# stephaneguindon/phyml

Measured on AMD Instinct MI355X. Metric: M partial-lk site-updates/sec on full-tree Lk(), higher is better.
Workload: dtype f64

## Files before the change

include/phyhip.h:

```cpp
#ifndef PHYHIP_H
#define PHYHIP_H

#ifdef __cplusplus
extern "C" {
#endif

#define PHYHIP_SUCCESS                         0
#define PHYHIP_ERROR_GENERAL                  (-1)
#define PHYHIP_ERROR_OUT_OF_MEMORY            (-2)
#define PHYHIP_ERROR_UNIDENTIFIED_EXCEPTION   (-3)
#define PHYHIP_ERROR_UNINITIALIZED_INSTANCE   (-4)
#define PHYHIP_ERROR_OUT_OF_RANGE             (-5)
#define PHYHIP_ERROR_NO_RESOURCE              (-6)
#define PHYHIP_ERROR_NO_IMPLEMENTATION        (-7)
#define PHYHIP_ERROR_FLOATING_POINT           (-8)

#define PHYHIP_OP_NONE (-1)

#define PHYHIP_FLAG_SHARDED (1L << 40)
#define PHYHIP_UNIQUE_ID_BYTES 128
#define PHYHIP_FLAG_CLASS_AXIS (1L << 41)
#define PHYHIP_FLAG_GENERIC_LOOP (1L << 42)

typedef struct
// ... 169 lines not shown
int phyhip_profile_read_traffic(int instance, double *outReadBytes, double *outWriteBytes);
int phyhip_profile_read_eigen(int instance, double *outEigenLrMs, int *outEigenLrLaunches, double *outDlkMs, int *outDlkLaunches);
int phyhip_profile_read_node_posteriors(int instance, double *outKernelMs, int *outCalls);
int phyhip_profile_read_pairwise(int instance, double *outCountMs, double *outOptimiseMs, int *outCalls);
int phyhip_profile_read_support(int instance, double *outKernelMs, int *outCalls);

int phyhip_get_resident_stats(int instance, long long out[8]);

int phyhip_get_big_resident_stats(int instance, long long out[4]);

int phyhip_set_virtual_buffers(int instance, int minOperations);

int phyhip_get_virtual_stats(int instance, long long out[4]);

int phyhip_get_deferred_stats(int instance, long long out[4]);

int phyhip_set_chained_buffers(int instance, int minOperations);

int phyhip_get_chained_stats(int instance, long long out[4]);

int phyhip_get_record_stats(int instance, long long out[12]);

int phyhip_get_step_kind_stats(int instance, long long out[16]);

int phyhip_tip_row_bits(const unsigned char *codes, long long n);


typedef struct { int destination, child1, child2; } phyhip_parsimony_operation;

int phyhip_set_parsimony(int instance, int general, const int *stepMatrix);
int phyhip_update_partial_parsimony(int instance, const phyhip_parsimony_operation *ops, int count);
int phyhip_calculate_edge_parsimony(int instance, int buffer1, int buffer2, long long *outParsimony);
int phyhip_get_site_parsimony(int instance, int *outSitePars);
int phyhip_get_partial_parsimony(int instance, int bufferIndex, int *outUi, int *outPars, int *outPPars );
int phyhip_profile_read_parsimony(int instance, double *outKernelMs, int *outLaunches, double *outPatternUpdates);

typedef struct { int child1, child2, subtree; } phyhip_parsimony_candidate;
int phyhip_calculate_regraft_parsimony(int instance, const phyhip_parsimony_candidate *candidates, int count, int keepCandidate,
                                       long long *outParsimony );
int phyhip_get_regraft_site_parsimony(int instance, int *outSitePars );
int phyhip_get_regraft_partial_parsimony(int instance, int *outUi, int *outPars, int *outPPars );
int phyhip_profile_read_regraft_parsimony(int instance, double *outKernelMs, int *outCalls, long long *outCandidates);


#define PHYHIP_REGRAFT_SUBTREE_IS_LEFT 1
typedef struct
// ... 54 lines not shown
```

phyml_amd/capi.py:

```python
from __future__ import annotations

import ctypes as C
import os

import numpy as np

_HERE = os.path.dirname(os.path.abspath(__file__))
LIB_DIR = os.environ.get("PHYHIP_LIBDIR") or os.path.join(_HERE, "lib")
LIB_PATH = os.path.join(LIB_DIR, "libphyhip.so")


class PhyhipError(RuntimeError):
    code = None


class Operation(C.Structure):
    _fields_ = [("destinationPartials", C.c_int), ("destinationScaleWrite", C.c_int), ("destinationScaleRead", C.c_int),
                ("child1Partials", C.c_int), ("child1TransitionMatrix", C.c_int),
                ("child2Partials", C.c_int), ("child2TransitionMatrix", C.c_int)]


class RegraftCandidate(C.Structure):
    _fields_ = [("child1Partials", C.c_int), ("child2Partials", C.c_int), ("subtreePartials", C.c_int), ("flags", C.c_int),
                ("child1Length", C.c_double), ("child2Length", C.c_double), ("subtreeLength", C.c_double)]
# ... 12 lines not shown
                ("evaluations", C.c_int * 3), ("status", C.c_int * 3), ("warning", C.c_int), ("reserved", C.c_int)]

    def as_tuple(self):
        return (tuple(self.length), self.lnL, self.dLnL, tuple(self.lkBegin), tuple(self.evaluations), tuple(self.status), self.warning)


class InstanceDetails(C.Structure):
    _fields_ = [("resourceNumber", C.c_int), ("resourceName", C.c_char * 64), ("implName", C.c_char * 64),
                ("flags", C.c_long), ("computeUnits", C.c_int), ("globalMemBytes", C.c_longlong)]


SYMBOLS = [
    "phyhip_create_instance", "phyhip_finalize_instance", "phyhip_get_last_error", "phyhip_set_tip_partials",
    "phyhip_set_tip_states", "phyhip_set_tip_partials_at_pattern", "phyhip_set_partials", "phyhip_set_pattern_weights", "phyhip_set_category_rates",
    "phyhip_set_category_weights", "phyhip_set_state_frequencies", "phyhip_set_eigen_decomposition",
    "phyhip_set_phyml_options", "phyhip_set_invariant_sites", "phyhip_update_transition_matrices",
    "phyhip_set_transition_matrix", "phyhip_get_transition_matrix", "phyhip_update_partials",
    "phyhip_calculate_edge_log_likelihoods", "phyhip_calculate_edge_log_likelihoods_device",
    "phyhip_get_site_log_likelihoods", "phyhip_get_site_outputs", "phyhip_get_partials", "phyhip_get_scale_factors",
    "phyhip_set_scale_factors", "phyhip_get_numerical_warning", "phyhip_update_eigen_lr",
    "phyhip_calculate_eigen_lnl_dlnl", "phyhip_calculate_eigen_lnl", "phyhip_get_dot_prod", "phyhip_set_stream",
    "phyhip_synchronize", "phyhip_profile", "phyhip_profile_read", "phyhip_calculate_mixture_log_likelihood",
    "phyhip_calculate_mixture_eigen_lnl_dlnl", "phyhip_comm_get_unique_id", "phyhip_comm_init_rank", "phyhip_comm_size",
    "phyhip_get_shard_range", "phyhip_profile_read_kernel", "phyhip_profile_read_collective", "phyhip_profile_read_traffic", "phyhip_profile_read_eigen", "phyhip_get_resident_stats", "phyhip_get_big_resident_stats", "phyhip_set_virtual_buffers", "phyhip_get_virtual_stats", "phyhip_get_deferred_stats", "phyhip_set_chained_buffers", "phyhip_get_chained_stats", "phyhip_get_record_stats", "phyhip_get_step_kind_stats", "phyhip_tip_row_bits", "phyhip_calculate_class_mixture_log_likelihood",
    "phyhip_calculate_class_mixture_eigen_lnl_dlnl", "phyhip_get_class_scale_factors", "phyhip_set_mixture_invariant_sites",
    "phyhip_calculate_edge_site_outputs_exact", "phyhip_calculate_node_state_posteriors", "phyhip_profile_read_node_posteriors",
    "phyhip_calculate_pairwise_ml_distances", "phyhip_set_pairwise_work_space", "phyhip_profile_read_pairwise",
    "phyhip_set_support_site_log_likelihoods", "phyhip_calculate_sh_support", "phyhip_get_support_alias_table", "phyhip_profile_read_support",
    "phyhip_set_parsimony", "phyhip_update_partial_parsimony", "phyhip_calculate_edge_parsimony", "phyhip_get_site_parsimony",
    "phyhip_get_partial_parsimony", "phyhip_profile_read_parsimony",
    "phyhip_calculate_regraft_parsimony", "phyhip_get_regraft_site_parsimony", "phyhip_get_regraft_partial_parsimony",
    "phyhip_profile_read_regraft_parsimony",
    "phyhip_optimise_edge_length", "phyhip_profile_read_edge_length",
    "phyhip_calculate_regraft_log_likelihoods", "phyhip_get_regraft_partials", "phyhip_get_regraft_transition_matrix",
    "phyhip_set_regraft_work_space", "phyhip_profile_read_regraft",
    "phyhip_calculate_mixture_regraft_log_likelihoods", "phyhip_get_mixture_regraft_partials",
    "phyhip_get_mixture_regraft_transition_matrix", "phyhip_set_mixture_regraft_work_space", "phyhip_profile_read_mixture_regraft",
    "phyhip_optimise_triples", "phyhip_get_triple_partials", "phyhip_set_triple_work_space", "phyhip_profile_read_triples",
]

FLAG_SHARDED = 1 << 40
FLAG_CLASS_AXIS = 1 << 41
UNIQUE_ID_BYTES = 128
PARS_TILE = 256
PARS_STAGING = 4096
MAX_PARS = 1000000000
PARS_REGRAFT_SLAB_FACTOR = 8
# ... 535 lines not shown
    def deferred_stats(self):
        out = (C.c_longlong * 4)()
        _chk(self.L.phyhip_get_deferred_stats(self.id, out))
        return tuple(int(v) for v in out)

    def set_chained_buffers(self, min_operations):
        _chk(self.L.phyhip_set_chained_buffers(self.id, int(min_operations)))

    def chained_stats(self):
        out = (C.c_longlong * 4)()
        _chk(self.L.phyhip_get_chained_stats(self.id, out))
        return tuple(int(v) for v in out)

    def record_stats(self):
        out = (C.c_longlong * 12)()
        _chk(self.L.phyhip_get_record_stats(self.id, out))
        return tuple(int(v) for v in out)

    def step_kind_stats(self):
        out = (C.c_longlong * 16)()
        _chk(self.L.phyhip_get_step_kind_stats(self.id, out))
        return tuple(int(v) for v in out[:8]), tuple(int(v) for v in out[8:])

    def profile_read_eigen(self):
        a = C.c_double(0); an = C.c_int(0); b = C.c_double(0); bn = C.c_int(0)
        _chk(self.L.phyhip_profile_read_eigen(self.id, C.byref(a), C.byref(an), C.byref(b), C.byref(bn)))
        return (a.value, an.value), (b.value, bn.value)

    def profile_read_collective(self):
        ms = C.c_double(0); n = C.c_int(0); r = C.c_int(0)
        _chk(self.L.phyhip_profile_read_collective(self.id, C.byref(ms), C.byref(n), C.byref(r)))
        return ms.value, n.value, r.value

    def profile_read_kernel(self):
        buf = C.create_string_buffer(128)
        _chk(self.L.phyhip_profile_read_kernel(self.id, buf, 128))
        return buf.value.decode()

    def profile_read_traffic(self):
        r = C.c_double(0); w = C.c_double(0)
        _chk(self.L.phyhip_profile_read_traffic(self.id, C.byref(r), C.byref(w)))
        return r.value, w.value


def mixture_log_likelihood(instance_ids, parents, children, matrices, proba, r_mat_weight, e_frq_weight, r_sum, e_sum, sum_probas):
    L = load()
# ... 50 lines not shown
```

phyml_amd/csrc/phyhip.hip:

```cpp
#include "phyhip_host.hpp"
#include "phyhip_side.hpp"

namespace phyhip_host
{

int fail(int code, const char *fmt, ...)
{
  char    buf[512];
  va_list ap;
  va_start(ap, fmt);
  vsnprintf(buf, sizeof buf, fmt, ap);
  va_end(ap);
  g_err = buf;
  return code;
}

}

using namespace phyhip_host;

extern "C" {

const char *phyhip_get_last_error(void) { return g_err.c_str(); }

// ... 1284 lines not shown
  GET_INST(I, instance);
  const Unstored::Counters &c = I->unstored.counters(Unstored::kChained);
  out[0] = I->unstored.n(Unstored::kChained); out[1] = (long long)c.skipped; out[2] = (long long)c.material; out[3] = (long long)c.dropped;
  return PHYHIP_SUCCESS;
}

int phyhip_get_record_stats(int instance, long long out[12])
{
  if (Group *G = get_group(instance)) return phyhip_get_record_stats(G->sub_id[0], out);
  GET_INST(I, instance);
  memcpy(out, I->rec_stats, sizeof I->rec_stats);
  return PHYHIP_SUCCESS;
}

int phyhip_get_step_kind_stats(int instance, long long out[2 * 8])
{
  if (Group *G = get_group(instance)) return phyhip_get_step_kind_stats(G->sub_id[0], out);
  GET_INST(I, instance);
  static_assert(kNtStepKinds == 8, "out[2][8]");
  memcpy(out, I->step_kinds, sizeof I->step_kinds);
  return PHYHIP_SUCCESS;
}

int phyhip_profile_read_collective(int instance, double *outMs, int *outCount, int *outRanks)
{
  Group *G = get_group(instance);
  GET_INST(I, G ? G->sub_id[0] : instance);
  int rc = flush_sync(I);
  if (rc) return rc;
  if ((rc = collect_profile(I))) return rc;
  if (outMs) *outMs = I->prof_aux_ms[2];
  if (outCount) *outCount = I->prof_aux_n[2];
  const Collective *co = G ? G->co : I->co;
  if (outRanks) *outRanks = co ? co->nranks : 1;
  return PHYHIP_SUCCESS;
}

int phyhip_profile_read_kernel(int instance, char *outName, int capacity)
{
  Group *G = get_group(instance);
  GET_INST_RES(I, G ? G->sub_id[0] : instance);
  I_call.leave_query();
  if (!outName || capacity < 1) return fail(PHYHIP_ERROR_OUT_OF_RANGE, "no room for the kernel name");
  snprintf(outName, (size_t)capacity, "%s", I->prof_kernel);
  return PHYHIP_SUCCESS;
}
// ... 24 lines not shown
```

phyml_amd/csrc/phyhip_host.hpp:

```cpp
#pragma once
#include "../../include/phyhip.h"
#include "phyhip_kernels.hpp"
#include "phyhip_aa.hpp"
#include "phyhip_nt2.hpp"
#include "phyhip_big.hpp"
#include "phyhip_matrix_queue.hpp"

#include <rccl/rccl.h>

#include <cfloat>
#include <functional>
#include <cmath>
#include <cstdarg>
#include <cstdio>
#include <cstdlib>
#include <cstring>
#include <ctime>
#include <atomic>
#include <chrono>
#include <condition_variable>
#include <mutex>
#include <thread>
#include <string>
#include <unordered_map>
// ... 259 lines not shown
  int          big_streak = 0;
  unsigned long long rb_dlk_api = 0;
  int          cus = 256;
  Resident    *r_inflight = nullptr;
  DlkParams    r_static;
  TreeParams   rt_static;
  SentCommand  sent;
  bool         rt_skip = false;
  unsigned long long clean_epoch = 0, rt_epoch = 0;
  bool         touched_call = false;
  bool               stream_dirty = true, dirty_prev = true;
  unsigned long long stamp_seq = 0, clean_after = 0;
  unsigned long long model_epoch = 1;
  unsigned long long api_no = 0, eig_api_no = 0;
  bool               fenced_eval = false;
  int          wall_khz = 0;
  bool      host_sum   = true;
  void     *d_pmscratch = nullptr;
  int       pm_scratch_cap = 0;
  char     *d_ops      = nullptr;
  size_t    ops_slot_bytes = 0;
  int       ops_cap = 0, ops_slots = 4, ops_slot = 0;
  long long rec_stats[12] = {0};
  long long step_kinds[2][kNtStepKinds] = {{0}};
  std::vector<uint8_t>   h_tiprows;
  std::vector<long long> tip_namb, tip_n15;
  std::vector<unsigned>  last_exec_fl;
  int       grid = 0, grid_nt = 0, block_nt = 64;

  std::vector<DevOp>                     pending;
  Unstored                               unstored;
  bool                                   virt_inline = true;
  std::vector<InlineDef>                 pending_inl;
  std::vector<std::vector<InlineDef>>    slot_inl;
  MatrixTable<double>                    rebuilds;
  MatrixTable<const double *>            uploads;
  std::vector<unsigned char>             mat_in_queue;
  std::vector<std::vector<DevOp>>        slot_ops;
  std::vector<int>                       slot_kind;
  std::vector<uint32_t>                  masks;
  std::unordered_map<uint32_t, int>      mask_code;
  bool                                   masks_dirty = false;
  std::vector<double>                    h_rates, h_eval, h_evec, h_ivec;
  std::vector<double>                    h_model;
  std::vector<unsigned char>             h_model_set;
  std::vector<short>                     h_invar;
// ... 338 lines not shown
```

phyml_amd/csrc/phyhip_kernels.hpp:

```cpp
#pragma once

#include <hip/hip_runtime.h>
#include <stdint.h>

#include "phyhip_exp.hpp"
#include "phyhip_log.hpp"

namespace phyhip
{

typedef const __attribute__((address_space(3))) unsigned long long *ExpLdsTab;
#ifdef PHYHIP_OCML_EXP
__device__ __forceinline__ double dev_exp(const double x, const unsigned long long * = nullptr) { return exp(x); }
#else
__device__ __forceinline__ double dev_exp(const double x) { return phyhip_exp_ref(x, phyhip_exp_tab); }
__device__ __forceinline__ double dev_exp(const double x, const unsigned long long *lds)
{
  return lds ? phyhip_exp_ref(x, (ExpLdsTab)lds) : phyhip_exp_ref(x, phyhip_exp_tab);
}
#endif
__device__ __forceinline__ void exp_tab_to_lds(unsigned long long *lds, const int tid, const int nth)
{
  for (int i = tid; i < 256; i += nth) lds[i] = phyhip_exp_tab[i];
}
// ... 57 lines not shown
  unsigned pmx;
};
struct alignas(16) NtExec
{
  unsigned fl;
  unsigned dst_data;
  unsigned dst_scale;
  unsigned pad;
};
enum : unsigned
{
  kRecL1 = 1u, kRecL2 = 2u,
  kRecA1 = 4u, kRecA2 = 8u,
  kRecT1 = 16u, kRecT2 = 32u,
  kRecIn1 = 64u, kRecIn2 = 128u,
  kRecStore = 256u
};
constexpr unsigned kRecKindShift = 12u;
constexpr int      kNtStepKinds  = 8;
#ifndef PHYHIP_NT_KINDS
#define PHYHIP_NT_KINDS 0x7e
#endif
constexpr bool nt2_bodied(int C, int G, bool INL) { return G >= 2 && !(C == 4 && G == 2 && !INL) && !(C == 2 && G == 2 && INL); }

struct TreeParams
{
  double         *partials;
  int            *scales;
  const double   *wght;
  long long       P;
  long long       Ppad;
  int             perm;
  int             C;
  int             tip_count;
  int             apply_scaling;
  int             n_ops;
  int             last_dest;
  int             edge_eval;
  double             *dot_out;
  int             e_parent, e_child, e_pm;
  const double   *pi;
  const double   *cat_w;
  int             invar_model;
  double          pinvar;
  const short    *invar;
  double         *site_lnl;
// ... 1718 lines not shown
```

phyml_amd/csrc/phyhip_nt2.hpp:

```cpp
#pragma once
#ifndef PHYHIP_LOAD_AUX
#define PHYHIP_LOAD_AUX 2
#endif
#ifndef PHYHIP_STORE_AUX
#define PHYHIP_STORE_AUX 2
#endif

#include "phyhip_kernels.hpp"

namespace phyhip
{

typedef unsigned int u32x2 __attribute__((ext_vector_type(2)));

struct NtFresh
{
  const int    *idx;
  const double *len;
  const double *evec, *ivec, *eval, *rates;
  const int    *up_idx = nullptr;
  const double *up_val = nullptr;
  bool          up_sys = false;
  const unsigned long long *exp_lds = nullptr;
};

template <int C, int G, bool DBG, int ARGS, int DIST = 2, int NW = 1, bool LREC = false, bool INL = false, bool BODIES = false>
__device__ __forceinline__ void nt2_run(const TreeParams &q, const IssueRec *__restrict__ irec, const ExecRec *__restrict__ xrec,
                                        const double *pmats,
                                        const uint8_t *__restrict__ tip_codes, unsigned long long *dbg, const NtFresh fr,
                                        const unsigned tile, const unsigned tid, double *lds_dot, const unsigned rec_no = 0xffffffffu)
{
  __shared__ unsigned long long stamps[DBG ? 64 * 8 : 1];
  const bool stamper = DBG && tile == gridDim.x / 2 && tid == 0;
#define PHY_STAMP(k_, i_)                                                                                              \
  if (DBG)                                                                                                             \
  {                                                                                                                    \
    const unsigned long long t_ = __builtin_readcyclecounter();                                                        \
    if (stamper && (k_) < 64) stamps[(k_) * 8 + (i_)] = t_;                                                            \
  }
  static_assert(C % G == 0 && 64 % G == 0, "category groups must divide the categories and the wave");
  constexpr int S = 4, CL = C / G, CS = CL * S, PW = 64 / G;
  static_assert(!INL || (ARGS == 0 && DIST == 2 && NW == 1 && !LREC), "in-step tip x tip children: list form only");
  constexpr int NM = INL ? 4 : 2;
  __shared__ __attribute__((aligned(16))) double lds_all[NW][2][NM * C * 16];
  double (&lds_p)[2][NM * C * 16] = lds_all[NW > 1 ? (tid >> 6) : 0];

  const int      lane = NW > 1 ? (int)(tid & 63) : (int)tid;
  const int      grp  = lane / PW, pl = lane % PW;
  const int      c0   = grp * CL;
  const unsigned p    = tile * (unsigned)PW + pl;
  constexpr int  HP   = CS / 2;
  const unsigned rowb = (unsigned)(q.Ppad * 16);
  const bool     cls    = (CL == 1) && q.class_axis != 0;
// ... 18 lines not shown
    if constexpr (ARGS != 0)
    {
#pragma unroll
      for (int d = PW; d < 64; d <<= 1) v = max(v, (unsigned)__shfl_xor((int)v, d, 64));
      return v;
    }
    if constexpr (G == 4)
    {
      const auto r = __builtin_amdgcn_permlane16_swap(v, v, false, false);
      v = max((unsigned)r[0], (unsigned)r[1]);
    }
    if constexpr (G >= 2)
    {
      const auto r = __builtin_amdgcn_permlane32_swap(v, v, false, false);
      v = max((unsigned)r[0], (unsigned)r[1]);
    }
    return v;
  };

  constexpr bool all = ARGS != 0;
  constexpr bool compact = ARGS == 0;
  using IRec = typename std::conditional<compact, NtIssue, IssueRec>::type;
  using XRec = typename std::conditional<compact, NtExec, ExecRec>::type;
  const unsigned data_bytes = (unsigned)q.Ppad * (unsigned)(C * S * 8), scale_bytes = (unsigned)q.Ppad * (cls ? 4u * C : 4u), tip_bytes = (unsigned)q.Ppad;
  auto arena = [&](const void *base, unsigned off16, unsigned bytes) {
    const unsigned long long a = (unsigned long long)reinterpret_cast<uintptr_t>(base) + ((unsigned long long)uni(off16) << 4);
    return __builtin_amdgcn_make_buffer_rsrc(reinterpret_cast<void *>(a), 0, (int)bytes, 0x00020000);
  };
  auto compact_data = [&](const NtIssue &o, Raw &r) {
    const unsigned f = uni(o.fl);
    if (f & kRecL1)
    {
      const __amdgpu_buffer_rsrc_t d1r = arena(q.partials, o.data[0], data_bytes);
#pragma unroll
      for (int e = 0; e < HP; ++e) r.a[e] = __builtin_amdgcn_raw_buffer_load_b128(d1r, voff16, (unsigned)e * rowb, PHYHIP_LOAD_AUX);
    }
    if (f & kRecL2)
    {
      const __amdgpu_buffer_rsrc_t d2r = arena(q.partials, o.data[1], data_bytes);
#pragma unroll
      for (int e = 0; e < HP; ++e) r.b[e] = __builtin_amdgcn_raw_buffer_load_b128(d2r, voff16, (unsigned)e * rowb, PHYHIP_LOAD_AUX);
    }
    auto aux = [&](const bool tip, const unsigned off16) {
      const void *base = tip ? (const void *)tip_codes : (const void *)q.scales;
      return __builtin_amdgcn_raw_buffer_load_b32(arena(base, off16, tip ? tip_bytes : scale_bytes), tip ? (p & ~3u) : voff4, 0, 0);
    };
    if (f & kRecA1) r.sa = aux((f & kRecT1) != 0, o.aux[0]);
    if (f & kRecA2) r.sb = aux((f & kRecT2) != 0, o.aux[1]);
    if constexpr (INL)
    {
      if (f & (kRecIn1 | kRecIn2)) r.tx = __builtin_amdgcn_raw_buffer_load_b32(arena(tip_codes, (f >> 8) * (tip_bytes >> 4), tip_bytes), p & ~3u, 0, 0);
    }
  };
  auto desc_data = [&](const IssueRec &o, Raw &r) {
    if (all || uni(o.c1_data.bytes))
    {
      const __amdgpu_buffer_rsrc_t d1r = rsrc(o.c1_data);
#pragma unroll
      for (int e = 0; e < HP; ++e) r.a[e] = __builtin_amdgcn_raw_buffer_load_b128(d1r, voff16, (unsigned)e * rowb, PHYHIP_LOAD_AUX);
    }
    if (all || uni(o.c2_data.bytes))
    {
      const __amdgpu_buffer_rsrc_t d2r = rsrc(o.c2_data);
#pragma unroll
      for (int e = 0; e < HP; ++e) r.b[e] = __builtin_amdgcn_raw_buffer_load_b128(d2r, voff16, (unsigned)e * rowb, PHYHIP_LOAD_AUX);
    }
    if (all || uni(o.c1_scale.bytes)) r.sa = __builtin_amdgcn_raw_buffer_load_b32(rsrc(o.c1_scale), uni(o.c1_scale.x) ? (p & ~3u) : voff4, 0, 0);
    if (all || uni(o.c2_scale.bytes)) r.sb = __builtin_amdgcn_raw_buffer_load_b32(rsrc(o.c2_scale), uni(o.c2_scale.x) ? (p & ~3u) : voff4, 0, 0);
    if constexpr (INL)
    {
      const bool second = uni(o.c2_tip.x) != 0;
      if (second || uni(o.c1_tip.x) != 0)
      {
        Desc ct;
        ct.base = second ? o.c2_tip.base : o.c1_tip.base; ct.bytes = second ? o.c2_tip.bytes : o.c1_tip.bytes; ct.x = 0;
// ... 108 lines not shown
  auto IR = [&](int i) -> IRec {
    if constexpr (compact) return reinterpret_cast<const NtIssue *>(irec)[i];
    else if constexpr (ARGS != 0 && !LREC) return i ? q.arg_ir[1] : q.arg_ir[0];
    else return irec[i];
  };
  auto XR = [&](int i) -> XRec {
    if constexpr (compact) return reinterpret_cast<const NtExec *>(xrec)[i];
    else if constexpr (ARGS != 0 && !LREC) return i ? q.arg_xr[1] : q.arg_xr[0];
    else return xrec[i];
  };
  const int last = ARGS ? 1 : q.n_ops - 1;
  Raw       RA, RB;
  u32x4     PA, PB, PA2, PB2;
  if constexpr (!all)
  {
    const u32x4 z = {0u, 0u, 0u, 0u};
#pragma unroll
    for (int e = 0; e < HP; ++e) RA.a[e] = RA.b[e] = RB.a[e] = RB.b[e] = z;
    RA.sa = RA.sb = RA.tx = RB.sa = RB.sb = RB.tx = 0u;
    PA2 = PB2 = z;
  }
  constexpr bool single  = ARGS == 1;
  const bool     has_ops = ARGS == 0 ? q.n_ops > 0 : ARGS != 3;
  if (has_ops)
  {
    issue_data(IR(0), RA);
    if constexpr (!single && DIST == 2) issue_data(IR((1 < last) ? 1 : last), RB);
  }
  u32x4    EX[HP], EY[HP];
  unsigned esl = 0, esr = 0;
  if constexpr (ARGS)
  {
    if (q.edge_eval)
    {
      const size_t bufsz = (size_t)q.Ppad * C * S;
      auto pre = [&](int idx, u32x4 (&v)[HP], unsigned &sc) {
        const u32x4 *src = reinterpret_cast<const u32x4 *>(q.partials + (size_t)(idx - q.tip_count) * bufsz) + (size_t)(c0 * 2) * q.Ppad + p;
#pragma unroll
        for (int e = 0; e < HP; ++e) v[e] = src[(size_t)e * q.Ppad];
        sc = (unsigned)q.scales[(size_t)(idx - q.tip_count) * (cls ? C : 1) * q.Ppad + voff4 / 4];
      };
      if (q.e_prefetch & 1) pre(q.e_parent, EX, esl);
      if (q.e_prefetch & 2) pre(q.e_child, EY, esr);
    }
  }

  if (q.n_up > 0)
// ... 529 lines not shown
          if (iv >= 0) invariant_lk(inv, issue_, q.pi[iv], f, q.apply_scaling);
          if (issue_) { f = 0; site = q.pi[iv] * q.pinvar; }
          else site = site * (1. - q.pinvar) + inv * q.pinvar;
        }
        if (site < kSmall) { site = kSmall; raise_warn(q); }
        const double lsl = log(site) - kLog2 * (double)f;
        if (q.site_lnl) q.site_lnl[p] = lsl;
        if (q.site_lk) q.site_lk[p] = dev_exp(lsl);
        contrib = w * lsl;
      }
      q.fact[p] = f;
    }
  }
#pragma unroll
  for (int off = 32; off > 0; off >>= 1) contrib += __shfl_down(contrib, off, 64);
  if (LREC && q.tile_sums == tile_sums_in_wave())
  {
    if (lane == 0) lds_dot[tile / (unsigned)(NW * kBigGroupWgs)] = contrib;
    return;
  }
  publish_block_sum(q, contrib, lane, rec_no == 0xffffffffu ? tile : rec_no);
}

template <int C, int G = 1, bool DBG = false, int ARGS = 0, int DIST = 2, bool INL = false>
__global__ __launch_bounds__(64, DIST == 1 ? G + 1 : G) void traverse_nt2_kernel(const TreeParams q, const IssueRec *__restrict__ irec,
                                                             const ExecRec *__restrict__ xrec, const double *pmats,
                                                             const uint8_t *__restrict__ tip_codes,
                                                             unsigned long long *dbg = nullptr)
{
  typedef const __attribute__((address_space(4))) char karg_char;
  const char *ka = (const char *)(karg_char *)__builtin_amdgcn_kernarg_segment_ptr();
  NtFresh     fr;
  fr.idx  = reinterpret_cast<const int *>(ka + offsetof(TreeParams, fresh_idx));
  fr.len  = reinterpret_cast<const double *>(ka + offsetof(TreeParams, fresh_len));
  fr.evec = reinterpret_cast<const double *>(ka + offsetof(TreeParams, m_evec));
  fr.ivec = reinterpret_cast<const double *>(ka + offsetof(TreeParams, m_ivec));
  fr.eval = reinterpret_cast<const double *>(ka + offsetof(TreeParams, m_eval));
  fr.rates = reinterpret_cast<const double *>(ka + offsetof(TreeParams, m_rates));
  fr.up_idx = reinterpret_cast<const int *>(ka + offsetof(TreeParams, up_idx));
  fr.up_val = reinterpret_cast<const double *>(ka + offsetof(TreeParams, up_val));
  __shared__ __attribute__((aligned(16))) double lds_dot[(64 / G) * C * 4];
  nt2_run<C, G, DBG, ARGS, DIST, 1, false, INL, ARGS == 0 && DIST == 2 && nt2_bodied(C, G, INL)>(q, irec, xrec, pmats, tip_codes, dbg, fr, blockIdx.x, threadIdx.x, lds_dot);
}

template <int C, bool INL>
__global__ __launch_bounds__(64, 2) void traverse_nt2_mixed_kernel(const TreeParams q, const IssueRec *__restrict__ irec,
                                                                   const ExecRec *__restrict__ xrec, const double *pmats,
                                                                   const uint8_t *__restrict__ tip_codes, const int n2)
{
  static_assert(C == 4, "four-lane waves: one category per lane");
  typedef const __attribute__((address_space(4))) char karg_char;
  const char *ka = (const char *)(karg_char *)__builtin_amdgcn_kernarg_segment_ptr();
  NtFresh     fr;
  fr.idx  = reinterpret_cast<const int *>(ka + offsetof(TreeParams, fresh_idx));
  fr.len  = reinterpret_cast<const double *>(ka + offsetof(TreeParams, fresh_len));
  fr.evec = reinterpret_cast<const double *>(ka + offsetof(TreeParams, m_evec));
  fr.ivec = reinterpret_cast<const double *>(ka + offsetof(TreeParams, m_ivec));
  fr.eval = reinterpret_cast<const double *>(ka + offsetof(TreeParams, m_eval));
  fr.rates = reinterpret_cast<const double *>(ka + offsetof(TreeParams, m_rates));
  fr.up_idx = reinterpret_cast<const int *>(ka + offsetof(TreeParams, up_idx));
  fr.up_val = reinterpret_cast<const double *>(ka + offsetof(TreeParams, up_val));
  __shared__ __attribute__((aligned(16))) double lds_dot[32 * C * 4];
  if ((int)blockIdx.x < n2)
    nt2_run<C, 2, false, 0, 2, 1, false, INL, true>(q, irec, xrec, pmats, tip_codes, nullptr, fr, blockIdx.x, threadIdx.x, lds_dot);
  else
    nt2_run<C, 4, false, 0, 2, 1, false, INL, true>(q, irec, xrec, pmats, tip_codes, nullptr, fr, 2u * (unsigned)n2 + (blockIdx.x - (unsigned)n2),
                                              threadIdx.x, lds_dot, blockIdx.x);
}

constexpr int kResidentNtWords = 10 + 2 * 12;

template <int C, int G>
__global__ __launch_bounds__(64, 1) void resident_nt2_kernel(const TreeParams sq, const ResidentCtl r, const double *pmats,
                                                             const uint8_t *__restrict__ tip_codes, const double *evec,
                                                             const double *ivec, const double *eval, const double *rates)
{
  __shared__ unsigned long long sh_raw[64];
  __shared__ int                sh_idx[4];
  __shared__ double             sh_len[4];
  __shared__ __attribute__((aligned(16))) double sh_dot[(64 / G) * C * 4];
  __shared__ unsigned long long sh_exp[256];
  const int          lane = threadIdx.x;
  unsigned long long last = r.start_seq, t_last = wall_clock64();
  bool               mail_open = false;
  exp_tab_to_lds(sh_exp, lane, 64);
  __builtin_amdgcn_wave_barrier();
  for (;;)
  {
    const int act = resident_poll_wave(r, last, t_last, mail_open, sh_raw, 1, lane, blockIdx.x == 0);
    if (act == 2) return;
// ... 48 lines not shown
```

phyml_amd/csrc/phyhip_queue.hip:

```cpp
#include "phyhip_host.hpp"
#include <algorithm>

namespace phyhip_host
{

int flush_uploads(Instance *I)
{
  const auto &up = I->uploads;
  if (!up.empty())
  {
    big_release(I);
    I->touched_call = true;
  }
  size_t done = 0;
  while (done < up.size())
  {
    const int n = (int)std::min<size_t>(up.size() - done, kUploadBatch);
    MatUploadParams q;
    memset(&q, 0, sizeof q);
    q.count = n; q.S = I->S; q.C = I->C; q.pmats = I->d_pmats; q.afrag = I->perm ? I->d_afrag : nullptr;
    for (int k = 0; k < kUploadBatch; ++k) q.shadow[k] = -1;
    for (int k = 0; k < n; ++k) { q.idx[k] = up.idx()[done + k]; q.src[k] = up.payload()[done + k]; q.shadow[k] = up.snapshot()[done + k]; }
    hipLaunchKernelGGL(upload_matrices_kernel, dim3(n), dim3(256), q.afrag ? sizeof(double) * (size_t)I->C * I->S * I->S : 0, I->stream, q);
    HIPCHK(hipGetLastError());
// ... 274 lines not shown
    fl |= child_descs(I, o.c1, false, e1, e2, (unsigned)o.pm1 * matbytes, matbytes, (o.pad & kOpInl1) ? inl : nullptr, ir[k].c1_data, ir[k].c1_scale, ir[k].c1_tip);
    fl |= child_descs(I, o.c2, true, e1, e2, (unsigned)o.pm2 * matbytes, matbytes, (o.pad & kOpInl2) ? inl : nullptr, ir[k].c2_data, ir[k].c2_scale, ir[k].c2_tip);
    const size_t b = (size_t)(o.dest - I->tips);
    const bool   st_on = !(o.pad & kOpNoStore);
    xr[k].dst_data  = make_desc(I->d_partials + b * buf_elems(I), st_on ? bufbytes : 0, fl);
    xr[k].dst_scale = make_desc(I->d_scales + b * scale_elems(I), st_on ? scale_elems(I) * 4 : 0, 0);
    if (I->perm && f.has_inl)
    {
      const unsigned long long ab = inl ? ((unsigned long long)((unsigned)inl->pmA * matbytes) | ((unsigned long long)((unsigned)inl->pmB * matbytes) << 32)) : 0ull;
      ir[k].c1_tip = make_desc(reinterpret_cast<const void *>((uintptr_t)ab), (size_t)f.aa_need[k], inl ? ((o.pad & kOpInl1) ? 1u : 2u) : 0u);
      ir[k].c2_tip = make_desc(I->d_tipmasks + (size_t)(inl ? inl->b : 0) * I->Ppad, inl ? (size_t)I->Ppad * 4 : 0, (unsigned)f.aa_slot[k]);
      xr[k].dst_scale.x = (unsigned)f.aa_slot[k];
    }
  }
}

static bool compact_list_form(const Instance *I)
{
  if (!I->soa || I->perm) return false;
  const int g = I->nt_groups;
  return (I->C == 1 && g == 1) || (I->C == 2 && g <= 2) || (I->C == 3 && g == 1) || (I->C == 4 && (g == 1 || g == 2 || g == 4));
}

static int fill_compact_records(Instance *I, const FlushPlan &f, NtIssue *ir, NtExec *xr, int n_rec)
{
  const int    n_ops = f.n_ops;
  const size_t data16 = buf_elems(I) * sizeof(double) / 16, scale16 = scale_elems(I) * 4 / 16, tip16 = (size_t)I->Ppad / 16;
  const size_t n_int = (size_t)(I->nbuf - I->tips);
  if (n_int * data16 > 0xffffffffull || (size_t)I->tips * tip16 > 0xffffffffull || I->tips >= (1 << 24))
    return fail(PHYHIP_ERROR_OUT_OF_RANGE, "an arena of this instance is beyond the reach of a record's offset (64 GiB, 2^24 tips)");
  const unsigned matbytes = (unsigned)((size_t)I->C * I->S * I->S * sizeof(double));
  auto at = [&](int k) -> const DevOp & { return I->pending[std::min(k, n_ops - 1)]; };
  long long (&kinds)[2][5] = *reinterpret_cast<long long (*)[2][5]>(I->rec_stats + 2);
  const bool mixed  = I->mix_n4 > 0 && I->C == 4 && I->nt_groups == 2 && !I->ablate;
  const bool bodied = I->prefetch_dist == 2 && I->nt_groups >= 2 && (mixed || nt2_bodied(I->C, I->nt_groups, f.has_inl));
  ++I->rec_stats[0];
  for (int k = 0; k < n_rec; ++k)
  {
    const DevOp     &o  = at(k);
    const int        e1 = k >= 1 ? at(k - 1).dest : -1;
    const int        e2 = (k >= 2 && I->prefetch_dist == 2) ? at(k - 2).dest : -1;
    const InlineDef *inl = (o.pad & (kOpInl1 | kOpInl2)) ? &I->pending_inl[std::min(k, n_ops - 1)] : nullptr;
    NtIssue          r;
    memset(&r, 0, sizeof r);
    unsigned fl = 0;
    int      how[2] = {-1, -1};
    auto     onehot = [&](int tip) { return (tip_row_bits(I, tip) & 1) != 0; };
    auto child = [&](int c, int s, int pm, bool in_step) {
      r.pm[s] = (unsigned)pm * matbytes;
      if (in_step)
      {
        if (onehot(inl->a) && onehot(inl->b)) how[s] = 2;
        r.fl |= (kRecIn1 | kRecA1 | kRecT1) << s | (unsigned)inl->b << 8;
        r.data[s] = (unsigned)inl->pmA * matbytes; r.pmx = (unsigned)inl->pmB * matbytes;
        r.aux[s] = (unsigned)((size_t)inl->a * tip16);
        fl |= kOpCh1 << s;
        ++kinds[s][1];
        return;
      }
      const size_t b = (size_t)(c - I->tips);
      if (c < I->tips) { r.fl |= (kRecA1 | kRecT1) << s; r.aux[s] = (unsigned)((size_t)c * tip16); fl |= kOpTip1 << s; ++kinds[s][0]; if (onehot(c)) how[s] = 0; }
      else if (c == e1) { fl |= s ? kOpF21 : kOpF11; ++kinds[s][2]; how[s] = 1; }
      else if (c == e2) { fl |= s ? kOpF22 : kOpF12; ++kinds[s][3]; }
      else
      {
        if (!I->no_loads) { r.fl |= (kRecL1 | kRecA1) << s; r.data[s] = (unsigned)(b * data16); r.aux[s] = (unsigned)(b * scale16); }
        ++kinds[s][4];
      }
    };
    child(o.c1, 0, o.pm1, inl && (o.pad & kOpInl1));
    child(o.c2, 1, o.pm2, inl && (o.pad & kOpInl2));
    ir[k] = r;
    static const unsigned char kind_of[3][3] = {{0, 1, 6}, {2, 0, 4}, {5, 3, 0}};
    unsigned kind = (how[0] >= 0 && how[1] >= 0) ? kind_of[how[0]][how[1]] : 0u;
    if (!((PHYHIP_NT_KINDS >> kind) & 1) || !bodied) kind = 0;
    ++I->step_kinds[k & 1][kind];
    fl |= kind << kRecKindShift;
    const size_t b = (size_t)(o.dest - I->tips);
    xr[k].fl = fl | ((o.pad & kOpNoStore) ? 0u : kRecStore);
    xr[k].dst_data = (unsigned)(b * data16); xr[k].dst_scale = (unsigned)(b * scale16); xr[k].pad = 0;
    if (kDiag) { I->last_exec_fl.resize((size_t)n_rec); I->last_exec_fl[(size_t)k] = xr[k].fl; }
  }
  return 0;
}

static int build_op_records(Instance *I, FlushPlan &f, TreeParams &q)
{
  const int  n_ops = f.n_ops;
  const bool fat = f.fat;
  q.last_dest = -1;
  if (n_ops == 0) return 0;
  const bool   compact = fat && compact_list_form(I) && !f.big_cmd();
  const int    kind = fat ? (compact ? 16 : 0) + I->prefetch_dist : 0, n_rec = n_ops + (n_ops & 1);
  const size_t ib = (compact ? sizeof(NtIssue) : sizeof(IssueRec)) * n_rec, xb = (compact ? sizeof(NtExec) : sizeof(ExecRec)) * n_rec;
  int          hit = -1, rc = 0;
  for (int sl = 0; sl < I->ops_slots && hit < 0; ++sl)
    if (I->slot_kind[sl] == kind && I->slot_ops[sl].size() == (size_t)n_ops &&
        memcmp(I->slot_ops[sl].data(), I->pending.data(), sizeof(DevOp) * n_ops) == 0 && I->slot_inl[sl] == I->pending_inl)
      hit = sl;
  const bool in_args = hit < 0 && fat && (I->soa || I->perm) && I->args_recs && n_ops <= 2;
  char      *dst = I->d_ops + (size_t)(hit >= 0 ? hit : I->ops_slot) * I->ops_slot_bytes;
  int        new_slot = -1;
  if (hit < 0)
  {
    const size_t bytes = fat ? ib + xb : sizeof(DevOp) * n_ops;
    void        *st = nullptr;
    if (!in_args)
    {
      new_slot = I->ops_slot;
      I->slot_kind[new_slot] = -1;
      if (bytes > I->ops_slot_bytes)
        return fail(PHYHIP_ERROR_OUT_OF_RANGE, "a launch of %d %s does not fit a device slot of %zu bytes", fat ? n_rec : n_ops,
                    fat ? "operation records" : "operations", I->ops_slot_bytes);
      if ((rc = I->ring.alloc(bytes, I->stream, &st))) return rc;
    }
    if (!fat) memcpy(st, I->pending.data(), bytes);
// ... 770 lines not shown
```

Baseline: 51880.

## Stage tip code rows in LDS table for NT2 compact traversal kernel

At kernel start, each block loads the tip-code rows for its tile (up to 256 tips) into a shared-memory table. Compact records now mark tip children with table flags and a tip index instead of a global offset, so per-step tip loads become LDS reads, and buffer loads are skipped when a record needs no memory. This is meant to take scattered global tip-code loads off the per-operation critical path. In exchange it adds a prologue that loads all table rows, uses more LDS (which can lower occupancy), narrows the tip-index field to 20 bits, and adds a stats query.

Result: faster. 53880, median of 5 (+3.9%).

```diff
diff --git a/include/phyhip.h b/include/phyhip.h
--- a/include/phyhip.h
+++ b/include/phyhip.h
@@ -215,6 +215,8 @@
 int phyhip_get_record_stats(int instance, long long out[12]);
 
 int phyhip_get_step_kind_stats(int instance, long long out[16]);
+
+int phyhip_get_tip_table_stats(int instance, long long out[4]);
 
 int phyhip_tip_row_bits(const unsigned char *codes, long long n);
 
diff --git a/phyml_amd/capi.py b/phyml_amd/capi.py
--- a/phyml_amd/capi.py
+++ b/phyml_amd/capi.py
@@ -58,7 +58,7 @@
     "phyhip_calculate_eigen_lnl_dlnl", "phyhip_calculate_eigen_lnl", "phyhip_get_dot_prod", "phyhip_set_stream",
     "phyhip_synchronize", "phyhip_profile", "phyhip_profile_read", "phyhip_calculate_mixture_log_likelihood",
     "phyhip_calculate_mixture_eigen_lnl_dlnl", "phyhip_comm_get_unique_id", "phyhip_comm_init_rank", "phyhip_comm_size",
-    "phyhip_get_shard_range", "phyhip_profile_read_kernel", "phyhip_profile_read_collective", "phyhip_profile_read_traffic", "phyhip_profile_read_eigen", "phyhip_get_resident_stats", "phyhip_get_big_resident_stats", "phyhip_set_virtual_buffers", "phyhip_get_virtual_stats", "phyhip_get_deferred_stats", "phyhip_set_chained_buffers", "phyhip_get_chained_stats", "phyhip_get_record_stats", "phyhip_get_step_kind_stats", "phyhip_tip_row_bits", "phyhip_calculate_class_mixture_log_likelihood",
+    "phyhip_get_shard_range", "phyhip_profile_read_kernel", "phyhip_profile_read_collective", "phyhip_profile_read_traffic", "phyhip_profile_read_eigen", "phyhip_get_resident_stats", "phyhip_get_big_resident_stats", "phyhip_set_virtual_buffers", "phyhip_get_virtual_stats", "phyhip_get_deferred_stats", "phyhip_set_chained_buffers", "phyhip_get_chained_stats", "phyhip_get_record_stats", "phyhip_get_step_kind_stats", "phyhip_get_tip_table_stats", "phyhip_tip_row_bits", "phyhip_calculate_class_mixture_log_likelihood",
     "phyhip_calculate_class_mixture_eigen_lnl_dlnl", "phyhip_get_class_scale_factors", "phyhip_set_mixture_invariant_sites",
     "phyhip_calculate_edge_site_outputs_exact", "phyhip_calculate_node_state_posteriors", "phyhip_profile_read_node_posteriors",
     "phyhip_calculate_pairwise_ml_distances", "phyhip_set_pairwise_work_space", "phyhip_profile_read_pairwise",
@@ -640,6 +640,11 @@
         _chk(self.L.phyhip_get_step_kind_stats(self.id, out))
         return tuple(int(v) for v in out[:8]), tuple(int(v) for v in out[8:])
 
+    def tip_table_stats(self):
+        out = (C.c_longlong * 4)()
+        _chk(self.L.phyhip_get_tip_table_stats(self.id, out))
+        return tuple(int(v) for v in out)
+
     def profile_read_eigen(self):
         a = C.c_double(0); an = C.c_int(0); b = C.c_double(0); bn = C.c_int(0)
         _chk(self.L.phyhip_profile_read_eigen(self.id, C.byref(a), C.byref(an), C.byref(b), C.byref(bn)))
diff --git a/phyml_amd/csrc/phyhip.hip b/phyml_amd/csrc/phyhip.hip
--- a/phyml_amd/csrc/phyhip.hip
+++ b/phyml_amd/csrc/phyhip.hip
@@ -1330,6 +1330,14 @@
   return PHYHIP_SUCCESS;
 }
 
+int phyhip_get_tip_table_stats(int instance, long long out[4])
+{
+  if (Group *G = get_group(instance)) return phyhip_get_tip_table_stats(G->sub_id[0], out);
+  GET_INST(I, instance);
+  memcpy(out, I->tip_tab_stats, sizeof I->tip_tab_stats);
+  return PHYHIP_SUCCESS;
+}
+
 int phyhip_profile_read_collective(int instance, double *outMs, int *outCount, int *outRanks)
 {
   Group *G = get_group(instance);
diff --git a/phyml_amd/csrc/phyhip_host.hpp b/phyml_amd/csrc/phyhip_host.hpp
--- a/phyml_amd/csrc/phyhip_host.hpp
+++ b/phyml_amd/csrc/phyhip_host.hpp
@@ -305,6 +305,7 @@
   size_t    ops_slot_bytes = 0;
   int       ops_cap = 0, ops_slots = 4, ops_slot = 0;
   long long rec_stats[12] = {0};
+  long long tip_tab_stats[4] = {0};
   long long step_kinds[2][kNtStepKinds] = {{0}};
   std::vector<uint8_t>   h_tiprows;
   std::vector<long long> tip_namb, tip_n15;
diff --git a/phyml_amd/csrc/phyhip_kernels.hpp b/phyml_amd/csrc/phyhip_kernels.hpp
--- a/phyml_amd/csrc/phyhip_kernels.hpp
+++ b/phyml_amd/csrc/phyhip_kernels.hpp
@@ -103,6 +103,18 @@
 #define PHYHIP_NT_KINDS 0x7e
 #endif
 constexpr bool nt2_bodied(int C, int G, bool INL) { return G >= 2 && !(C == 4 && G == 2 && !INL) && !(C == 2 && G == 2 && INL); }
+
+constexpr int kNtTabTips = 256;
+#ifndef PHYHIP_NT_TIPTAB
+#define PHYHIP_NT_TIPTAB 1
+#endif
+constexpr unsigned kRecTipShift = 8u, kRecTipBits = 20u;
+enum : unsigned
+{
+  kRecTab1 = 1u << 28, kRecTab2 = 1u << 29, kRecTabX = 1u << 30, kRecAny = 1u << 31
+};
+__host__ __device__ constexpr int nt_tab_rows(long long Ppad, int tips) { return Ppad > (1ll << 23) ? 0 : (tips < kNtTabTips ? tips : kNtTabTips); }
+constexpr bool nt2_tabbed(int C, int G, bool INL) { return PHYHIP_NT_TIPTAB != 0 && nt2_bodied(C, G, INL) && !(C == 4 && G == 2 && INL); }
 
 struct TreeParams
 {
diff --git a/phyml_amd/csrc/phyhip_nt2.hpp b/phyml_amd/csrc/phyhip_nt2.hpp
--- a/phyml_amd/csrc/phyhip_nt2.hpp
+++ b/phyml_amd/csrc/phyhip_nt2.hpp
@@ -24,11 +24,12 @@
   const unsigned long long *exp_lds = nullptr;
 };
 
-template <int C, int G, bool DBG, int ARGS, int DIST = 2, int NW = 1, bool LREC = false, bool INL = false, bool BODIES = false>
+template <int C, int G, bool DBG, int ARGS, int DIST = 2, int NW = 1, bool LREC = false, bool INL = false, bool BODIES = false, bool TAB = false>
 __device__ __forceinline__ void nt2_run(const TreeParams &q, const IssueRec *__restrict__ irec, const ExecRec *__restrict__ xrec,
                                         const double *pmats,
                                         const uint8_t *__restrict__ tip_codes, unsigned long long *dbg, const NtFresh fr,
-                                        const unsigned tile, const unsigned tid, double *lds_dot, const unsigned rec_no = 0xffffffffu)
+                                        const unsigned tile, const unsigned tid, double *lds_dot, const unsigned rec_no = 0xffffffffu,
+                                        unsigned *tip_tab = nullptr)
 {
   __shared__ unsigned long long stamps[DBG ? 64 * 8 : 1];
   const bool stamper = DBG && tile == gridDim.x / 2 && tid == 0;
@@ -93,13 +94,31 @@
   constexpr bool compact = ARGS == 0;
   using IRec = typename std::conditional<compact, NtIssue, IssueRec>::type;
   using XRec = typename std::conditional<compact, NtExec, ExecRec>::type;
+  constexpr bool tabbed = TAB && BODIES && compact && G >= 2 && DIST == 2;
+  const unsigned *tab_lane = tabbed ? tip_tab + (pl >> 2) : nullptr;
   const unsigned data_bytes = (unsigned)q.Ppad * (unsigned)(C * S * 8), scale_bytes = (unsigned)q.Ppad * (cls ? 4u * C : 4u), tip_bytes = (unsigned)q.Ppad;
   auto arena = [&](const void *base, unsigned off16, unsigned bytes) {
     const unsigned long long a = (unsigned long long)reinterpret_cast<uintptr_t>(base) + ((unsigned long long)uni(off16) << 4);
     return __builtin_amdgcn_make_buffer_rsrc(reinterpret_cast<void *>(a), 0, (int)bytes, 0x00020000);
   };
-  auto compact_data = [&](const NtIssue &o, Raw &r) {
+  auto compact_tab = [&](const NtIssue &o, Raw &r) {
+    if constexpr (tabbed)
+    {
+      const unsigned f = uni(o.fl);
+      if (f & kRecTab1) r.sa = tab_lane[uni(o.aux[0]) * (unsigned)(PW / 4)];
+      if (f & kRecTab2) r.sb = tab_lane[uni(o.aux[1]) * (unsigned)(PW / 4)];
+      if constexpr (INL)
+      {
+        if (f & kRecTabX) r.tx = tab_lane[((f >> kRecTipShift) & ((1u << kRecTipBits) - 1u)) * (unsigned)(PW / 4)];
+      }
+    }
+  };
+  auto compact_mem = [&](const NtIssue &o, Raw &r) {
     const unsigned f = uni(o.fl);
+    if constexpr (tabbed)
+    {
+      if (!(f & kRecAny)) return;
+    }
     if (f & kRecL1)
     {
       const __amdgpu_buffer_rsrc_t d1r = arena(q.partials, o.data[0], data_bytes);
@@ -120,8 +139,13 @@
     if (f & kRecA2) r.sb = aux((f & kRecT2) != 0, o.aux[1]);
     if constexpr (INL)
     {
-      if (f & (kRecIn1 | kRecIn2)) r.tx = __builtin_amdgcn_raw_buffer_load_b32(arena(tip_codes, (f >> 8) * (tip_bytes >> 4), tip_bytes), p & ~3u, 0, 0);
-    }
+      const unsigned second = tabbed ? (f >> kRecTipShift) & ((1u << kRecTipBits) - 1u) : f >> 8;
+      if ((f & (kRecIn1 | kRecIn2)) && !(tabbed && (f & kRecTabX))) r.tx = __builtin_amdgcn_raw_buffer_load_b32(arena(tip_codes, second * (tip_bytes >> 4), tip_bytes), p & ~3u, 0, 0);
+    }
+  };
+  auto compact_data = [&](const NtIssue &o, Raw &r) {
+    compact_tab(o, r);
+    compact_mem(o, r);
   };
   auto desc_data = [&](const IssueRec &o, Raw &r) {
     if (all || uni(o.c1_data.bytes))
@@ -276,7 +300,35 @@
   }
   constexpr bool single  = ARGS == 1;
   const bool     has_ops = ARGS == 0 ? q.n_ops > 0 : ARGS != 3;
-  if (has_ops)
+  if constexpr (tabbed)
+  {
+    if (has_ops)
+    {
+      constexpr int DW = PW / 4, RP = 64 / DW, NP = kNtTabTips / RP, GP = 8;
+      static_assert(NP % GP == 0, "passes come in groups");
+      const int                    n_rows = nt_tab_rows(q.Ppad, q.tip_count);
+      const __amdgpu_buffer_rsrc_t tr = __builtin_amdgcn_make_buffer_rsrc(const_cast<uint8_t *>(tip_codes), 0, n_rows * (int)q.Ppad, 0x00020000);
+      const unsigned               foff = (unsigned)(lane / DW) * (unsigned)q.Ppad + tile * (unsigned)PW + (unsigned)(lane % DW) * 4u;
+      unsigned                     tv[NP];
+#pragma unroll
+      for (int g = 0; g < NP / GP; ++g)
+        if (g * GP * RP < n_rows)
+#pragma unroll
+          for (int i = 0; i < GP; ++i)
+            tv[g * GP + i] = __builtin_amdgcn_raw_buffer_load_b32(tr, foff + (unsigned)((g * GP + i) * RP) * (unsigned)q.Ppad, 0, 0);
+      compact_mem(IR(0), RA);
+      compact_mem(IR((1 < last) ? 1 : last), RB);
+#pragma unroll
+      for (int g = 0; g < NP / GP; ++g)
+        if (g * GP * RP < n_rows)
+#pragma unroll
+          for (int i = 0; i < GP; ++i) tip_tab[(g * GP + i) * 64 + lane] = tv[g * GP + i];
+      __builtin_amdgcn_wave_barrier();
+      compact_tab(IR(0), RA);
+      compact_tab(IR((1 < last) ? 1 : last), RB);
+    }
+  }
+  else if (has_ops)
   {
     issue_data(IR(0), RA);
     if constexpr (!single && DIST == 2) issue_data(IR((1 < last) ? 1 : last), RB);
@@ -852,6 +904,19 @@
   publish_block_sum(q, contrib, lane, rec_no == 0xffffffffu ? tile : rec_no);
 }
 
+template <bool ON, int BYTES> struct NtTipTab
+{
+  static __device__ __forceinline__ unsigned *get()
+  {
+    __shared__ unsigned tab[BYTES / 4];
+    return tab;
+  }
+};
+template <int BYTES> struct NtTipTab<false, BYTES>
+{
+  static __device__ __forceinline__ unsigned *get() { return nullptr; }
+};
+
 template <int C, int G = 1, bool DBG = false, int ARGS = 0, int DIST = 2, bool INL = false>
 __global__ __launch_bounds__(64, DIST == 1 ? G + 1 : G) void traverse_nt2_kernel(const TreeParams q, const IssueRec *__restrict__ irec,
                                                              const ExecRec *__restrict__ xrec, const double *pmats,
@@ -870,7 +935,10 @@
   fr.up_idx = reinterpret_cast<const int *>(ka + offsetof(TreeParams, up_idx));
   fr.up_val = reinterpret_cast<const double *>(ka + offsetof(TreeParams, up_val));
   __shared__ __attribute__((aligned(16))) double lds_dot[(64 / G) * C * 4];
-  nt2_run<C, G, DBG, ARGS, DIST, 1, false, INL, ARGS == 0 && DIST == 2 && nt2_bodied(C, G, INL)>(q, irec, xrec, pmats, tip_codes, dbg, fr, blockIdx.x, threadIdx.x, lds_dot);
+  constexpr bool bodied = ARGS == 0 && DIST == 2 && nt2_bodied(C, G, INL);
+  constexpr bool tabbed = bodied && nt2_tabbed(C, G, INL);
+  nt2_run<C, G, DBG, ARGS, DIST, 1, false, INL, bodied, tabbed>(q, irec, xrec, pmats, tip_codes, dbg, fr, blockIdx.x, threadIdx.x, lds_dot, 0xffffffffu,
+                                                                NtTipTab<tabbed, (64 / G) * kNtTabTips>::get());
 }
 
 template <int C, bool INL>
@@ -891,11 +959,13 @@
   fr.up_idx = reinterpret_cast<const int *>(ka + offsetof(TreeParams, up_idx));
   fr.up_val = reinterpret_cast<const double *>(ka + offsetof(TreeParams, up_val));
   __shared__ __attribute__((aligned(16))) double lds_dot[32 * C * 4];
+  constexpr bool tabbed = PHYHIP_NT_TIPTAB != 0;
+  unsigned      *tab = NtTipTab<tabbed, 32 * kNtTabTips>::get();
   if ((int)blockIdx.x < n2)
-    nt2_run<C, 2, false, 0, 2, 1, false, INL, true>(q, irec, xrec, pmats, tip_codes, nullptr, fr, blockIdx.x, threadIdx.x, lds_dot);
+    nt2_run<C, 2, false, 0, 2, 1, false, INL, true, tabbed>(q, irec, xrec, pmats, tip_codes, nullptr, fr, blockIdx.x, threadIdx.x, lds_dot, 0xffffffffu, tab);
   else
-    nt2_run<C, 4, false, 0, 2, 1, false, INL, true>(q, irec, xrec, pmats, tip_codes, nullptr, fr, 2u * (unsigned)n2 + (blockIdx.x - (unsigned)n2),
-                                              threadIdx.x, lds_dot, blockIdx.x);
+    nt2_run<C, 4, false, 0, 2, 1, false, INL, true, tabbed>(q, irec, xrec, pmats, tip_codes, nullptr, fr, 2u * (unsigned)n2 + (blockIdx.x - (unsigned)n2),
+                                              threadIdx.x, lds_dot, blockIdx.x, tab);
 }
 
 constexpr int kResidentNtWords = 10 + 2 * 12;
diff --git a/phyml_amd/csrc/phyhip_queue.hip b/phyml_amd/csrc/phyhip_queue.hip
--- a/phyml_amd/csrc/phyhip_queue.hip
+++ b/phyml_amd/csrc/phyhip_queue.hip
@@ -320,18 +320,32 @@
   return (I->C == 1 && g == 1) || (I->C == 2 && g <= 2) || (I->C == 3 && g == 1) || (I->C == 4 && (g == 1 || g == 2 || g == 4));
 }
 
+static bool nt_list_bodied(const Instance *I, bool has_inl)
+{
+  const bool mixed = I->mix_n4 > 0 && I->C == 4 && I->nt_groups == 2 && !I->ablate;
+  return I->prefetch_dist == 2 && I->nt_groups >= 2 && (mixed || nt2_bodied(I->C, I->nt_groups, has_inl));
+}
+
+static int nt_tip_table(const Instance *I, bool has_inl)
+{
+  if (PHYHIP_NT_TIPTAB == 0 || !nt_list_bodied(I, has_inl)) return 0;
+  const bool mixed = I->mix_n4 > 0 && I->C == 4 && I->nt_groups == 2 && !I->ablate;
+  return mixed || nt2_tabbed(I->C, I->nt_groups, has_inl) ? nt_tab_rows(I->Ppad, I->tips) : 0;
+}
+
 static int fill_compact_records(Instance *I, const FlushPlan &f, NtIssue *ir, NtExec *xr, int n_rec)
 {
   const int    n_ops = f.n_ops;
   const size_t data16 = buf_elems(I) * sizeof(double) / 16, scale16 = scale_elems(I) * 4 / 16, tip16 = (size_t)I->Ppad / 16;
   const size_t n_int = (size_t)(I->nbuf - I->tips);
-  if (n_int * data16 > 0xffffffffull || (size_t)I->tips * tip16 > 0xffffffffull || I->tips >= (1 << 24))
-    return fail(PHYHIP_ERROR_OUT_OF_RANGE, "an arena of this instance is beyond the reach of a record's offset (64 GiB, 2^24 tips)");
+  if (n_int * data16 > 0xffffffffull || (size_t)I->tips * tip16 > 0xffffffffull || I->tips >= (1 << kRecTipBits))
+    return fail(PHYHIP_ERROR_OUT_OF_RANGE, "an arena of this instance is beyond the reach of a record's offset (64 GiB, 2^20 tips)");
   const unsigned matbytes = (unsigned)((size_t)I->C * I->S * I->S * sizeof(double));
   auto at = [&](int k) -> const DevOp & { return I->pending[std::min(k, n_ops - 1)]; };
   long long (&kinds)[2][5] = *reinterpret_cast<long long (*)[2][5]>(I->rec_stats + 2);
-  const bool mixed  = I->mix_n4 > 0 && I->C == 4 && I->nt_groups == 2 && !I->ablate;
-  const bool bodied = I->prefetch_dist == 2 && I->nt_groups >= 2 && (mixed || nt2_bodied(I->C, I->nt_groups, f.has_inl));
+  const bool bodied = nt_list_bodied(I, f.has_inl);
+  const int  tab_rows = nt_tip_table(I, f.has_inl);
+  I->tip_tab_stats[0] = tab_rows ? kNtTabTips : 0; I->tip_tab_stats[3] = tab_rows ? (long long)kNtTabTips * (64 / I->nt_groups) : 0;
   ++I->rec_stats[0];
   for (int k = 0; k < n_rec; ++k)
   {
@@ -344,20 +358,28 @@
     unsigned fl = 0;
     int      how[2] = {-1, -1};
     auto     onehot = [&](int tip) { return (tip_row_bits(I, tip) & 1) != 0; };
+    auto tip_aux = [&](int tip, int s) {
+      const bool tab = tip < tab_rows;
+      ++I->tip_tab_stats[tab ? 1 : 2];
+      r.fl |= tab ? kRecTab1 << s : (kRecA1 | kRecT1) << s;
+      r.aux[s] = tab ? (unsigned)tip : (unsigned)((size_t)tip * tip16);
+    };
     auto child = [&](int c, int s, int pm, bool in_step) {
       r.pm[s] = (unsigned)pm * matbytes;
       if (in_step)
       {
         if (onehot(inl->a) && onehot(inl->b)) how[s] = 2;
-        r.fl |= (kRecIn1 | kRecA1 | kRecT1) << s | (unsigned)inl->b << 8;
+        r.fl |= kRecIn1 << s | (unsigned)inl->b << kRecTipShift;
+        tip_aux(inl->a, s);
+        ++I->tip_tab_stats[inl->b < tab_rows ? 1 : 2];
+        if (inl->b < tab_rows) r.fl |= kRecTabX;
         r.data[s] = (unsigned)inl->pmA * matbytes; r.pmx = (unsigned)inl->pmB * matbytes;
-        r.aux[s] = (unsigned)((size_t)inl->a * tip16);
         fl |= kOpCh1 << s;
         ++kinds[s][1];
         return;
       }
       const size_t b = (size_t)(c - I->tips);
-      if (c < I->tips) { r.fl |= (kRecA1 | kRecT1) << s; r.aux[s] = (unsigned)((size_t)c * tip16); fl |= kOpTip1 << s; ++kinds[s][0]; if (onehot(c)) how[s] = 0; }
+      if (c < I->tips) { tip_aux(c, s); fl |= kOpTip1 << s; ++kinds[s][0]; if (onehot(c)) how[s] = 0; }
       else if (c == e1) { fl |= s ? kOpF21 : kOpF11; ++kinds[s][2]; how[s] = 1; }
       else if (c == e2) { fl |= s ? kOpF22 : kOpF12; ++kinds[s][3]; }
       else
@@ -368,6 +390,7 @@
     };
     child(o.c1, 0, o.pm1, inl && (o.pad & kOpInl1));
     child(o.c2, 1, o.pm2, inl && (o.pad & kOpInl2));
+    if (tab_rows && ((r.fl & (kRecL1 | kRecL2 | kRecA1 | kRecA2)) || ((r.fl & (kRecIn1 | kRecIn2)) && !(r.fl & kRecTabX)))) r.fl |= kRecAny;
     ir[k] = r;
     static const unsigned char kind_of[3][3] = {{0, 1, 6}, {2, 0, 4}, {5, 3, 0}};
     unsigned kind = (how[0] >= 0 && how[1] >= 0) ? kind_of[how[0]][how[1]] : 0u;
@@ -389,7 +412,7 @@
   q.last_dest = -1;
   if (n_ops == 0) return 0;
   const bool   compact = fat && compact_list_form(I) && !f.big_cmd();
-  const int    kind = fat ? (compact ? 16 : 0) + I->prefetch_dist : 0, n_rec = n_ops + (n_ops & 1);
+  const int    kind = fat ? (compact ? (nt_tip_table(I, f.has_inl) ? 32 : 16) : 0) + I->prefetch_dist : 0, n_rec = n_ops + (n_ops & 1);
   const size_t ib = (compact ? sizeof(NtIssue) : sizeof(IssueRec)) * n_rec, xb = (compact ? sizeof(NtExec) : sizeof(ExecRec)) * n_rec;
   int          hit = -1, rc = 0;
   for (int sl = 0; sl < I->ops_slots && hit < 0; ++sl)
```
